# lebrice/blurred-GAN

Measured on AMD Instinct MI355X. Metric: images/sec (G+D+GP step), higher is better.
Workload: dtype f32; 1 GPU; celeba64 64x64x3 batch 256/GPU, blur sigma 5.0 (31 taps), D-step+GP+G-step+Adam; global_batch=256, parallelism=dp1

## Files before the change

blurred-gan_amd/csrc/conv_rows.hip:

```cpp
#include "conv_common.h"
#include <algorithm>
#include <cstdlib>
#include <cstring>
#include <type_traits>

namespace {

typedef float floatx4 __attribute__((ext_vector_type(4)));

struct RowParams {
  const float* A;
  const float* Wt;
  float* C;
  int B, Hi, Wi, Ck, Ho, Wo, N;
  int pt, pl, flip;
  int R, strips;
  int wpr, ipw;
  int epi_mode;
  const float* bias;
  const float* ref;
  const unsigned char* keep;
  size_t keep_elems;
  float alpha, scale;
};

__device__ inline int floordiv(int a, int b) { return a >= 0 ? a / b : -((-a + b - 1) / b); }

__device__ inline float tanh_branchless(float x) {
  float ax = fabsf(x);
  ax = ax > 15.f ? 15.f : ax;
  const float e = __builtin_amdgcn_exp2f(ax * 2.885390081777927f);
  const float big = 1.f - 2.f * __builtin_amdgcn_rcpf(e + 1.f);
  const float x2 = ax * ax;
  const float small = ax * fmaf(x2, fmaf(x2, fmaf(x2, -17.f / 315.f, 2.f / 15.f), -1.f / 3.f), 1.f);
  return copysignf(ax < 0.1f ? small : big, x);
}

template <int KS, int K, int S, int PIXW, int EP>
__global__ __launch_bounds__(PIXW * 4) void conv_rows_scatter_kernel(const RowParams p) {
  constexpr int NTH = PIXW * 4;
  constexpr unsigned kOob = 0x80000000u;
  extern __shared__ __attribute__((aligned(16))) float row_lds[];
  constexpr int AS = 4 * KS + 4;
  float* abuf = row_lds;
  constexpr int PS = PIXW * 17 + 1;
  float* pbuf = row_lds + 2 * PIXW * AS;
  const int tid = threadIdx.x, lane = tid & 63, wave = tid >> 6;
  const int li = lane & 15, kq = lane >> 4;
  const int t = wave % p.wpr, img = wave / p.wpr;
  const int strip = blockIdx.x % p.strips, bgrp = blockIdx.x / p.strips;
  const int Ck = 4 * KS, N = p.N;
  const int y0 = strip * p.R, y1 = min(y0 + p.R, p.Ho);
  const int iy_lo = -floordiv(-(y0 + p.pt - (K - 1)), S);
  const int iy_hi = floordiv(y1 - 1 + p.pt, S);
  const int nrows = iy_hi - iy_lo + 1;
  const int nimg = min(p.ipw, p.B - bgrp * p.ipw);
  const size_t img0 = (size_t)bgrp * p.ipw;
  const __amdgpu_buffer_rsrc_t rsA = __builtin_amdgcn_make_buffer_rsrc(const_cast<float*>(p.A + img0 * p.Hi * p.Wi * Ck), 0,
                                                                        nimg * p.Hi * p.Wi * Ck * 4, 0x00020000);
  const __amdgpu_buffer_rsrc_t rsC = __builtin_amdgcn_make_buffer_rsrc(p.C + img0 * p.Ho * p.Wo * N, 0, nimg * p.Ho * p.Wo * N * 4, 0x00020000);

  float bw[K][KS];
  {
    const int lc = min(li, K * N - 1);
    const int kw = lc / N, n = lc - kw * N;
#pragma unroll
    for (int kh = 0; kh < K; ++kh) {
      const int tap = p.flip ? (K - 1 - kh) * K + (K - 1 - kw) : kh * K + kw;
#pragma unroll
      for (int ks = 0; ks < KS; ++ks) {
        const float w = p.Wt[((size_t)tap * N + n) * Ck + 4 * ks + kq];
        bw[kh][ks] = li < K * N ? w : 0.f;
      }
    }
  }
  floatx4 acc[K];
#pragma unroll
  for (int i = 0; i < K; ++i) acc[i] = floatx4{0.f, 0.f, 0.f, 0.f};

  constexpr int QPR = KS;
  constexpr int NQ = PIXW * QPR / NTH;
  static_assert(NQ >= 1, "Ck >= 16");
  unsigned g_off[NQ], l_off[NQ];
#pragma unroll
  for (int q = 0; q < NQ; ++q) {
    const int f = tid + q * NTH, pix = f / QPR, c4 = f - pix * QPR;
    const int im = pix / p.Wi, ix = pix - im * p.Wi;
    g_off[q] = im < nimg ? (unsigned)(((im * p.Hi * p.Wi + ix) * Ck + c4 * 4) * 4) : kOob;
    l_off[q] = (unsigned)(pix * AS + c4 * 4);
  }
  const int rowB = p.Wi * Ck * 4;
  auto gload = [&](int r, float4 (&g)[NQ]) {
    const int iy = iy_lo + r;
    const bool row_ok = r < nrows && (unsigned)iy < (unsigned)p.Hi;
    const unsigned add = row_ok ? (unsigned)(iy * rowB) : 0u, force = row_ok ? 0u : kOob;
#pragma unroll
    for (int q = 0; q < NQ; ++q)
      g[q] = __builtin_bit_cast(float4, __builtin_amdgcn_raw_buffer_load_b128(rsA, (g_off[q] + add) | force, 0, 0));
  };
  auto lstore = [&](int buf, const float4 (&g)[NQ]) {
#pragma unroll
    for (int q = 0; q < NQ; ++q) *reinterpret_cast<float4*>(abuf + (size_t)buf * PIXW * AS + l_off[q]) = g[q];
  };
  const float* afrag = abuf + ((size_t)img * p.Wi + 16 * t + li) * AS + kq;
  constexpr int NE = (S * (16 / K) + 3) / 4;
  constexpr int NTERM = (K + S - 1) / S;
  int e_src[NE][NTERM];
  unsigned e_dst[NE];
  float e_bias[NE], e_mul[NE];
  int e_n[NE];
  if (tid < 2 * S) pbuf[(size_t)tid * PS + PIXW * 17] = 0.f;
  {
    const int per_img = p.Wo * N;
#pragma unroll
    for (int q = 0; q < NE; ++q) {
      const int e = tid + q * NTH;
      const int im = e / per_img, rem = e - im * per_img;
      const int x = rem / N, n = rem - x * N;
      const bool ok = e < p.ipw * per_img && im < nimg;
      e_dst[q] = ok ? (unsigned)(((im * p.Ho * p.Wo + x) * N + n) * 4) : kOob;
      e_n[q] = n;
      e_bias[q] = ok && p.bias ? p.bias[n] : 0.f;
      e_mul[q] = ok && p.epi_mode == BG_EPI_AFFINE_LRELU ? p.ref[n] : 0.f;
#pragma unroll
      for (int i = 0; i < NTERM; ++i) {
        const int kw = (x + p.pl) % S + i * S;
        const int num = x + p.pl - kw, ix = num / S;
        e_src[q][i] = (ok && kw < K && num >= 0 && ix < p.Wi) ? (im * p.Wi + ix) * 17 + kw * N + n : PIXW * 17;
      }
    }
  }
  const size_t out0 = img0 * p.Ho * p.Wo * N;
  auto pwrite = [&](const floatx4& pacc, int slot) {
    float* pb = pbuf + (size_t)slot * PS;
#pragma unroll
    for (int rr = 0; rr < 4; ++rr) pb[((size_t)img * p.Wi + 16 * t + 4 * kq + rr) * 17 + li] = pacc[rr];
  };
  auto pstore = [&](int slot, int y, bool live) {
    const float* pb = pbuf + (size_t)slot * PS;
    float v[NE];
#pragma unroll
    for (int q = 0; q < NE; ++q) {
      v[q] = pb[e_src[q][0]];
#pragma unroll
      for (int i = 1; i < NTERM; ++i) v[q] += pb[e_src[q][i]];
    }
    const unsigned add = live ? (unsigned)(y * p.Wo * N * 4) : 0u, force = live ? 0u : kOob;
#pragma unroll
    for (int q = 0; q < NE; ++q) {
      const unsigned off = (e_dst[q] + add) | force;
      float o;
      if (EP == 0) {
        o = v[q] + e_bias[q];
      } else if (EP == 1) {
        o = tanh_branchless(v[q] + e_bias[q]);
      } else {
        const bool mine = (off & kOob) == 0;
        o = mine ? bg::apply_epilogue_pre(p, v[q], out0 + (off >> 2), e_bias[q], e_mul[q]) : 0.f;
      }
      __builtin_amdgcn_raw_buffer_store_b32(__builtin_bit_cast(unsigned, o), rsC, off, 0, 0);
    }
  };

  float4 g0[NQ], g1[NQ], g2[NQ], g3[NQ];
  gload(0, g0);
  gload(1, g1);
  gload(2, g2);
  gload(3, g3);
  lstore(0, g0);
  gload(4, g0);
#pragma unroll
  for (int i = 0; i < 4 * NE * S; ++i) __builtin_amdgcn_raw_buffer_store_b32(0u, rsC, kOob + 4u * i, 0, 0);
  int y_prev = 0;
  bool have_prev = false;
  auto flush_prev = [&](int prev_par) {
#pragma unroll
    for (int kh = 0; kh < S; ++kh) {
      const int y = y_prev + kh;
      pstore(prev_par * S + kh, y, have_prev & (y >= y0) & (y < y1));
    }
  };
  auto trip = [&](int r, auto parity, float4 (&g)[NQ]) {
    constexpr int cur = decltype(parity)::value;
    __syncthreads();
    float a[KS];
#pragma unroll
    for (int ks = 0; ks < KS; ++ks) a[ks] = afrag[(size_t)cur * PIXW * AS + 4 * ks];
#pragma unroll
    for (int ks = 0; ks < KS; ++ks)
#pragma unroll
      for (int kh = 0; kh < K; ++kh) acc[kh] = __builtin_amdgcn_mfma_f32_16x16x4f32(a[ks], bw[kh][ks], acc[kh], 0, 0, 0);
    flush_prev(cur ^ 1);
    lstore(cur ^ 1, g);
    gload(r + 5, g);
#pragma unroll
    for (int kh = 0; kh < S; ++kh) pwrite(acc[kh], cur * S + kh);
    y_prev = (iy_lo + r) * S - p.pt;
    have_prev = true;
#pragma unroll
    for (int i = 0; i < K; ++i) acc[i] = i + S < K ? acc[i + S] : floatx4{0.f, 0.f, 0.f, 0.f};
  };
  int r = 0;
  for (; r + 4 <= nrows; r += 4) {
    trip(r, std::integral_constant<int, 0>{}, g1);
    trip(r + 1, std::integral_constant<int, 1>{}, g2);
    trip(r + 2, std::integral_constant<int, 0>{}, g3);
    trip(r + 3, std::integral_constant<int, 1>{}, g0);
  }
  int last_par = 1;
  if (r < nrows) {
    trip(r, std::integral_constant<int, 0>{}, g1);
    last_par = 0;
    if (r + 1 < nrows) {
      trip(r + 1, std::integral_constant<int, 1>{}, g2);
      last_par = 1;
      if (r + 2 < nrows) {
        trip(r + 2, std::integral_constant<int, 0>{}, g3);
        last_par = 0;
      }
    }
  }
  __syncthreads();
  if (last_par == 0) flush_prev(0); else flush_prev(1);
}

template <int K, int S>
int launch_rows(const RowParams& p, dim3 grid, size_t lds, hipStream_t s) {
  const bool wide = p.Wi == 128;
  const int ep = p.epi_mode == BG_EPI_NONE ? 0 : p.epi_mode == BG_EPI_TANH ? 1 : 2;
#define BG_RS2(KSv, EPv) do { if (wide) bg::launch((conv_rows_scatter_kernel<KSv, K, S, 128, EPv>), grid, dim3(512), lds, s, p); \
                              else bg::launch((conv_rows_scatter_kernel<KSv, K, S, 64, EPv>), grid, dim3(256), lds, s, p); } while (0)
#define BG_RS(KSv) do { if (ep == 0) BG_RS2(KSv, 0); else if (ep == 1) BG_RS2(KSv, 1); else BG_RS2(KSv, 2); } while (0)
  switch (p.Ck) {
    case 16: BG_RS(4); return 1;
    case 32: BG_RS(8); return 1;
    case 64: BG_RS(16); return 1;
    default: return 0;
  }
#undef BG_RS
#undef BG_RS2
}

constexpr int kRgHalo = 16;

struct RowGParams {
  const float* A;
  const float* Wt;
  float* C;
  int B, Hi, Wi, Ct, Ho, Wo, N;
  int s, pt, pl, flip;
  int R, strips;
  int epi_mode;
  const float* bias;
  const float* ref;
  const unsigned char* keep;
  size_t keep_elems;
  float alpha, scale;
};

template <int TG, int NT, int K, bool MASK>
__global__ __launch_bounds__(256) void conv_rows_gather_kernel(const RowGParams p) {
  extern __shared__ __attribute__((aligned(16))) float xl[];
  const int tid = threadIdx.x, lane = tid & 63, wave = tid >> 6;
  const int li = lane & 15, kq = lane >> 4;
  const int Ct = p.Ct, N = 16 * NT, st = p.s;
  const int RS = p.Wi * Ct + 2 * kRgHalo;
  const int strip = blockIdx.x % p.strips, b = blockIdx.x / p.strips;
  const int oy0 = strip * p.R, rows = min(p.R, p.Ho - oy0);
  const int nrows_in = (rows - 1) * st + K;

  float bw[K][4][NT];
#pragma unroll
  for (int ks = 0; ks < 4; ++ks) {
    const int i = 4 * ks + kq, kw = i / Ct, ci = i - kw * Ct;
#pragma unroll
    for (int kh = 0; kh < K; ++kh) {
      const int tap = p.flip ? (K - 1 - kh) * K + (K - 1 - kw) : kh * K + kw;
#pragma unroll
      for (int nt = 0; nt < NT; ++nt) bw[kh][ks][nt] = i < K * Ct ? p.Wt[((size_t)tap * N + nt * 16 + li) * Ct + ci] : 0.f;
    }
  }
  const int RL = p.Wi * Ct;
  if ((RL & 3) == 0) {
    const int q4 = RS / 4;
    bg::stage_rows_f4<4>(xl, nrows_in, q4, RS, tid, [&](int r, int c4) -> const float* {
      const int iy = oy0 * st - p.pt + r, e = c4 * 4 - kRgHalo;
      return ((unsigned)iy < (unsigned)p.Hi && (unsigned)e < (unsigned)RL) ? p.A + ((size_t)b * p.Hi + iy) * RL + e : nullptr;
    });
  } else {
    for (int idx = tid; idx < nrows_in * RS; idx += 256) {
      const int r = idx / RS, c = idx - r * RS;
      const int iy = oy0 * st - p.pt + r, e = c - kRgHalo;
      float v = 0.f;
      if ((unsigned)iy < (unsigned)p.Hi && (unsigned)e < (unsigned)RL) v = p.A[((size_t)b * p.Hi + iy) * RL + e];
      xl[idx] = v;
    }
  }
  __syncthreads();

  float e_bias[NT], e_mul[NT];
#pragma unroll
  for (int nt = 0; nt < NT; ++nt) {
    e_bias[nt] = p.bias ? p.bias[nt * 16 + li] : 0.f;
    e_mul[nt] = p.epi_mode == BG_EPI_AFFINE_LRELU ? p.ref[nt * 16 + li] : 1.f;
  }
  const int groups = p.Wo / (16 * TG);
  const int nunits = rows * groups;
  for (int u = wave; u < nunits; u += 4) {
    const int r = u / groups, g = u - r * groups;
    const int oy = oy0 + r, ox0 = g * 16 * TG;
    floatx4 acc[TG][NT];
#pragma unroll
    for (int tg = 0; tg < TG; ++tg)
#pragma unroll
      for (int nt = 0; nt < NT; ++nt) acc[tg][nt] = floatx4{0.f, 0.f, 0.f, 0.f};
    const float* abase = xl + (size_t)(r * st) * RS + kRgHalo + ((ox0 + li) * st - p.pl) * Ct + kq;
#pragma unroll
    for (int kh = 0; kh < K; ++kh) {
      float a[TG][4];
#pragma unroll
      for (int tg = 0; tg < TG; ++tg)
#pragma unroll
        for (int ks = 0; ks < 4; ++ks) a[tg][ks] = abase[(size_t)kh * RS + tg * 16 * st * Ct + 4 * ks];
#pragma unroll
      for (int ks = 0; ks < 4; ++ks)
#pragma unroll
        for (int tg = 0; tg < TG; ++tg)
#pragma unroll
          for (int nt = 0; nt < NT; ++nt) acc[tg][nt] = __builtin_amdgcn_mfma_f32_16x16x4f32(a[tg][ks], bw[kh][ks][nt], acc[tg][nt], 0, 0, 0);
    }
    constexpr bool mask_epi = MASK;
#pragma unroll
    for (int tg = 0; tg < TG; ++tg) {
      const size_t pix0 = ((size_t)b * p.Ho + oy) * p.Wo + ox0 + 16 * tg + 4 * kq;
      unsigned char e_keep[4][NT];
      if (mask_epi) {
#pragma unroll
        for (int rr = 0; rr < 4; ++rr)
#pragma unroll
          for (int nt = 0; nt < NT; ++nt) {
            const size_t idx = (pix0 + rr) * N + nt * 16 + li;
            e_keep[rr][nt] = p.keep[(p.keep_elems == 0 || idx < p.keep_elems) ? idx : 0];
          }
      }
#pragma unroll
      for (int rr = 0; rr < 4; ++rr)
#pragma unroll
        for (int nt = 0; nt < NT; ++nt) {
          const size_t idx = (pix0 + rr) * N + nt * 16 + li;
          if (mask_epi) {
            float v = acc[tg][nt][rr] + e_bias[nt];
            v = v > 0.f ? v : p.alpha * v;
            if (p.keep_elems == 0 || idx < p.keep_elems) v = e_keep[rr][nt] ? v * p.scale : 0.f;
            p.C[idx] = v;
          } else {
            p.C[idx] = bg::apply_epilogue_pre(p, acc[tg][nt][rr], idx, e_bias[nt], e_mul[nt]);
          }
        }
    }
  }
}

template <int K>
int launch_rows_gather(const RowGParams& p, int tg, dim3 grid, size_t lds, hipStream_t s) {
  const int nt = p.N / 16;
  const bool mask = p.epi_mode == BG_EPI_BIAS_LRELU && p.keep != nullptr;
#define BG_RG(TGv, NTv) do { if (mask) bg::launch((conv_rows_gather_kernel<TGv, NTv, K, true>), grid, dim3(256), lds, s, p); \
                             else bg::launch((conv_rows_gather_kernel<TGv, NTv, K, false>), grid, dim3(256), lds, s, p); } while (0)
  if (tg == 1) { if (nt == 1) BG_RG(1, 1); else if (nt == 2) BG_RG(1, 2); else BG_RG(1, 4); }
  else if (tg == 2) { if (nt == 1) BG_RG(2, 1); else if (nt == 2) BG_RG(2, 2); else BG_RG(2, 4); }
  else { if (nt == 1) BG_RG(4, 1); else if (nt == 2) BG_RG(4, 2); else BG_RG(4, 4); }
#undef BG_RG
  return 1;
}

}

namespace bg {

int try_conv_rows_gather(int bwd_data, const float* a, const float* w, float* c, int B, int H, int W, int Cin, int Cout, int k, int s,
                         const bg_epilogue* epi, void* stream, int* taken) {
  *taken = 0;
  static const int off = getenv("BG_NO_ROWS") ? 1 : 0;
  if (off || (k != 5 && k != 3)) return BG_OK;
  RowGParams p;
  memset(&p, 0, sizeof p);
  int Ho, Wo, pt, pl;
  same_pads(H, k, s, &Ho, &pt);
  same_pads(W, k, s, &Wo, &pl);
  if (bwd_data) {
    if (s != 1 || Cout * k > 16 || (Cin != 16 && Cin != 32 && Cin != 64)) return BG_OK;
    p.Hi = H; p.Wi = W; p.Ct = Cout; p.Ho = H; p.Wo = W; p.N = Cin; p.s = 1; p.pt = k - 1 - pt; p.pl = k - 1 - pl; p.flip = 1;
  } else {
    if (Cin * k > 16 || (Cout != 16 && Cout != 32 && Cout != 64)) return BG_OK;
    p.Hi = H; p.Wi = W; p.Ct = Cin; p.Ho = Ho; p.Wo = Wo; p.N = Cout; p.s = s; p.pt = pt; p.pl = pl; p.flip = 0;
  }
  if (p.Wo % 16 != 0) return BG_OK;
  if ((size_t)B * p.Ho * p.Wo * p.N >= (1ull << 31)) return BG_OK;
  const int tiles = p.Wo / 16;
  const int tg = tiles % 4 == 0 ? 4 : (tiles % 2 == 0 ? 2 : 1);
  p.A = a; p.Wt = w; p.C = c; p.B = B;
  static const int rows_r = getenv("BG_ROWSG_R") ? atoi(getenv("BG_ROWSG_R")) : 0;
  p.R = std::min(rows_r ? rows_r : (s == 2 ? 8 : 16), p.Ho);
  p.strips = (int)cdiv(p.Ho, p.R);
  const size_t lds = ((size_t)((p.R - 1) * p.s + k) * (p.Wi * p.Ct + 2 * kRgHalo)) * sizeof(float);
  if (lds > 64 * 1024) return BG_OK;
  p.epi_mode = BG_EPI_NONE; p.alpha = 0.3f; p.scale = 1.f;
  if (epi) {
    BG_REQUIRE(epi->mode >= BG_EPI_NONE && epi->mode <= BG_EPI_AFFINE_LRELU, BG_ERR_UNSUPPORTED, "conv rows: epilogue mode %d", epi->mode);
    BG_REQUIRE(epi->mode != BG_EPI_MUL_GRAD || epi->ref, BG_ERR_NULL, "conv rows: BG_EPI_MUL_GRAD needs ref");
    BG_REQUIRE(epi->mode != BG_EPI_AFFINE_LRELU || (epi->ref && epi->bias), BG_ERR_NULL, "conv rows: BG_EPI_AFFINE_LRELU needs ref and bias");
    p.epi_mode = epi->mode; p.bias = epi->bias; p.ref = epi->ref; p.keep = epi->keep; p.keep_elems = epi->keep_elems; p.alpha = epi->alpha; p.scale = epi->scale;
  }
  const dim3 grid((unsigned)(B * p.strips));
  const double flops = 2.0 * B * (double)Ho * Wo * Cin * Cout * k * k;
  Launch L(stream, bwd_data ? "conv_rows_thin_k_dgrad" : "conv_rows_thin_k_fwd", flops, 0);
  if (k == 5) launch_rows_gather<5>(p, tg, grid, lds, L.s);
  else launch_rows_gather<3>(p, tg, grid, lds, L.s);
  *taken = 1;
  return L.done("conv_rows_gather_kernel");
}



int try_conv_rows(int bwd_data, const float* a, const float* w, float* c, int B, int H, int W, int Cin, int Cout, int k, int s,
                  const bg_epilogue* epi, void* stream, int* taken) {
  *taken = 0;
  static const int off = getenv("BG_NO_ROWS") ? 1 : 0;
  if (off || (k != 5 && k != 3)) return BG_OK;
  RowParams p;
  memset(&p, 0, sizeof p);
  int Ho, Wo, pt, pl;
  same_pads(H, k, s, &Ho, &pt);
  same_pads(W, k, s, &Wo, &pl);
  if (bwd_data) {
    if (Cin * k > 16 || (Cout != 16 && Cout != 32 && Cout != 64)) return BG_OK;
    p.Hi = Ho; p.Wi = Wo; p.Ck = Cout; p.Ho = H; p.Wo = W; p.N = Cin; p.pt = pt; p.pl = pl; p.flip = 0;
  } else {
    if (s != 1 || Cout * k > 16 || (Cin != 16 && Cin != 32 && Cin != 64)) return BG_OK;
    p.Hi = H; p.Wi = W; p.Ck = Cin; p.Ho = H; p.Wo = W; p.N = Cout; p.pt = k - 1 - pt; p.pl = k - 1 - pl; p.flip = 1;
  }
  if (p.Wi != 16 && p.Wi != 32 && p.Wi != 64 && p.Wi != 128) return BG_OK;
  if ((size_t)B * p.Hi * p.Wi * p.Ck >= (1ull << 31) || (size_t)B * p.Ho * p.Wo * p.N >= (1ull << 31)) return BG_OK;
  p.A = a; p.Wt = w; p.C = c; p.B = B;
  static const int rows_r = getenv("BG_ROWS_R") ? atoi(getenv("BG_ROWS_R")) : 0;
  p.R = std::min(rows_r ? rows_r : (s == 1 ? 32 : 16), p.Ho);
  p.strips = (int)cdiv(p.Ho, p.R);
  p.wpr = p.Wi / 16;
  p.ipw = p.Wi == 128 ? 1 : 4 / p.wpr;
  const int pixw = p.Wi == 128 ? 128 : 64;
  if ((long)p.ipw * p.Wo * p.N > (long)((s * (16 / k) + 3) / 4) * pixw * 4) return BG_OK;
  if ((size_t)p.ipw * p.Hi * p.Wi * p.Ck >= (1ull << 29) || (size_t)p.ipw * p.Ho * p.Wo * p.N >= (1ull << 29)) return BG_OK;
  p.epi_mode = BG_EPI_NONE; p.alpha = 0.3f; p.scale = 1.f;
  if (epi) {
    BG_REQUIRE(epi->mode >= BG_EPI_NONE && epi->mode <= BG_EPI_AFFINE_LRELU, BG_ERR_UNSUPPORTED, "conv rows: epilogue mode %d", epi->mode);
    BG_REQUIRE(epi->mode != BG_EPI_MUL_GRAD || epi->ref, BG_ERR_NULL, "conv rows: BG_EPI_MUL_GRAD needs ref");
    BG_REQUIRE(epi->mode != BG_EPI_AFFINE_LRELU || (epi->ref && epi->bias), BG_ERR_NULL, "conv rows: BG_EPI_AFFINE_LRELU needs ref and bias");
    p.epi_mode = epi->mode; p.bias = epi->bias; p.ref = epi->ref; p.keep = epi->keep; p.keep_elems = epi->keep_elems; p.alpha = epi->alpha; p.scale = epi->scale;
  }
  const dim3 grid((unsigned)(cdiv(B, p.ipw) * p.strips));
  const size_t lds = ((size_t)2 * pixw * (p.Ck + 4) + (size_t)2 * s * (pixw * 17 + 1)) * sizeof(float);
  const double flops = 2.0 * B * (double)H * W * Cin * Cout * k * k / (s * s);
  Launch L(stream, bwd_data ? "conv_rows_dgrad" : "conv_rows_fwd", flops, 0);
  int ok;
  if (k == 5) ok = s == 2 ? launch_rows<5, 2>(p, grid, lds, L.s) : launch_rows<5, 1>(p, grid, lds, L.s);
  else ok = s == 2 ? launch_rows<3, 2>(p, grid, lds, L.s) : launch_rows<3, 1>(p, grid, lds, L.s);
  (void)ok;
  *taken = 1;
  return L.done("conv_rows_scatter_kernel");
}

}
```

Baseline: 32500 images/s.

## Make thin-K row-gather conv persistent with double-buffered LDS prefetch and vector epilogues

Turns the row-gather conv into a persistent kernel sized from occupancy, and stages the next strip's input rows into registers while the current strip computes, then writes them into a second LDS buffer. Specialized epilogue variants (bias, bias+lrelu+dropout mask, mul-grad) use buffer loads and 128-bit stores with packed mask bytes instead of scalar per-element stores. It also transposes the MFMA operands so each lane holds four consecutive channels, enabling vector stores. The cost is doubled LDS usage, more template variants, extra alignment guards, and added register pressure.

```diff
diff --git a/blurred-gan_amd/csrc/conv_rows.hip b/blurred-gan_amd/csrc/conv_rows.hip
--- a/blurred-gan_amd/csrc/conv_rows.hip
+++ b/blurred-gan_amd/csrc/conv_rows.hip
@@ -2,11 +2,15 @@
 #include <algorithm>
 #include <cstdlib>
 #include <cstring>
+#include <map>
+#include <mutex>
 #include <type_traits>
+#include <utility>
 
 namespace {
 
 typedef float floatx4 __attribute__((ext_vector_type(4)));
+typedef unsigned uintx4 __attribute__((ext_vector_type(4)));
 
 struct RowParams {
   const float* A;
@@ -242,6 +246,11 @@
 }
 
 constexpr int kRgHalo = 16;
+constexpr int kRgPF = 4;
+constexpr int kRgBias = 0;
+constexpr int kRgLrelu = 1;
+constexpr int kRgMulGrad = 2;
+constexpr int kRgAny = 3;
 
 struct RowGParams {
   const float* A;
@@ -250,6 +259,9 @@
   int B, Hi, Wi, Ct, Ho, Wo, N;
   int s, pt, pl, flip;
   int R, strips;
+  int total;
+  int pre;
+  int ct_rcp;
   int epi_mode;
   const float* bias;
   const float* ref;
@@ -258,119 +270,231 @@
   float alpha, scale;
 };
 
-template <int TG, int NT, int K, bool MASK>
-__global__ __launch_bounds__(256) void conv_rows_gather_kernel(const RowGParams p) {
+template <int TG, int NT, int K, int EP>
+__global__ __launch_bounds__(256, (NT > 2 || EP == kRgAny) ? 1 : ((TG <= 2 || EP == kRgBias) ? 4 : 3)) void conv_rows_gather_kernel(const RowGParams p) {
+  constexpr unsigned kOob = 0x80000000u;
+  constexpr int N = 16 * NT;
   extern __shared__ __attribute__((aligned(16))) float xl[];
-  const int tid = threadIdx.x, lane = tid & 63, wave = tid >> 6;
+  const int tid = threadIdx.x, lane = tid & 63, wave = __builtin_amdgcn_readfirstlane(tid >> 6);
   const int li = lane & 15, kq = lane >> 4;
-  const int Ct = p.Ct, N = 16 * NT, st = p.s;
-  const int RS = p.Wi * Ct + 2 * kRgHalo;
-  const int strip = blockIdx.x % p.strips, b = blockIdx.x / p.strips;
-  const int oy0 = strip * p.R, rows = min(p.R, p.Ho - oy0);
-  const int nrows_in = (rows - 1) * st + K;
+  const int Ct = p.Ct, st = p.s;
+  const int RL = p.Wi * Ct;
+  const int RS = RL + 2 * kRgHalo;
+  const int nrmax = (p.R - 1) * st + K, bufsz = nrmax * RS;
+  constexpr bool pre = EP != kRgAny;
 
   float bw[K][4][NT];
-#pragma unroll
-  for (int ks = 0; ks < 4; ++ks) {
-    const int i = 4 * ks + kq, kw = i / Ct, ci = i - kw * Ct;
-#pragma unroll
-    for (int kh = 0; kh < K; ++kh) {
-      const int tap = p.flip ? (K - 1 - kh) * K + (K - 1 - kw) : kh * K + kw;
-#pragma unroll
-      for (int nt = 0; nt < NT; ++nt) bw[kh][ks][nt] = i < K * Ct ? p.Wt[((size_t)tap * N + nt * 16 + li) * Ct + ci] : 0.f;
-    }
-  }
-  const int RL = p.Wi * Ct;
-  if ((RL & 3) == 0) {
-    const int q4 = RS / 4;
-    bg::stage_rows_f4<4>(xl, nrows_in, q4, RS, tid, [&](int r, int c4) -> const float* {
-      const int iy = oy0 * st - p.pt + r, e = c4 * 4 - kRgHalo;
-      return ((unsigned)iy < (unsigned)p.Hi && (unsigned)e < (unsigned)RL) ? p.A + ((size_t)b * p.Hi + iy) * RL + e : nullptr;
-    });
-  } else {
-    for (int idx = tid; idx < nrows_in * RS; idx += 256) {
-      const int r = idx / RS, c = idx - r * RS;
-      const int iy = oy0 * st - p.pt + r, e = c - kRgHalo;
-      float v = 0.f;
-      if ((unsigned)iy < (unsigned)p.Hi && (unsigned)e < (unsigned)RL) v = p.A[((size_t)b * p.Hi + iy) * RL + e];
-      xl[idx] = v;
-    }
-  }
-  __syncthreads();
-
-  float e_bias[NT], e_mul[NT];
+  {
+    const __amdgpu_buffer_rsrc_t rsW = __builtin_amdgcn_make_buffer_rsrc(const_cast<float*>(p.Wt), 0, K * K * N * Ct * 4, 0x00020000);
+#pragma unroll
+    for (int ks = 0; ks < 4; ++ks) {
+      const int i = 4 * ks + kq, kw = (i * p.ct_rcp) >> 16, ci = i - kw * Ct;
+      const int kwt = p.flip ? K - 1 - kw : kw;
+      const unsigned vo = i < K * Ct ? (unsigned)(((kwt * N + li) * Ct + ci) * 4) : kOob;
+#pragma unroll
+      for (int kh = 0; kh < K; ++kh) {
+        const int kht = p.flip ? K - 1 - kh : kh;
+#pragma unroll
+        for (int nt = 0; nt < NT; ++nt)
+          bw[kh][ks][nt] = __builtin_bit_cast(float, __builtin_amdgcn_raw_buffer_load_b32(rsW, vo, (kht * K * N + nt * 16) * Ct * 4, 0));
+      }
+    }
+  }
+  float4 e_bias[NT], e_mul[NT];
 #pragma unroll
   for (int nt = 0; nt < NT; ++nt) {
-    e_bias[nt] = p.bias ? p.bias[nt * 16 + li] : 0.f;
-    e_mul[nt] = p.epi_mode == BG_EPI_AFFINE_LRELU ? p.ref[nt * 16 + li] : 1.f;
-  }
+    const int c = nt * 16 + 4 * kq;
+    e_bias[nt] = p.bias ? make_float4(p.bias[c], p.bias[c + 1], p.bias[c + 2], p.bias[c + 3]) : make_float4(0.f, 0.f, 0.f, 0.f);
+    e_mul[nt] = (EP == kRgAny && p.epi_mode == BG_EPI_AFFINE_LRELU) ? make_float4(p.ref[c], p.ref[c + 1], p.ref[c + 2], p.ref[c + 3])
+                                                                     : make_float4(1.f, 1.f, 1.f, 1.f);
+  }
+
+  unsigned gl_off[kRgPF];
+  if constexpr (pre) {
+    const int q4 = RL >> 2, dr = 256 / q4, dc = 256 - dr * q4;
+    int r = tid / q4, c4 = tid - r * q4;
+#pragma unroll
+    for (int i = 0; i < kRgPF; ++i) {
+      const unsigned packed = (unsigned)(r * q4 + c4) | ((unsigned)(r * (RS >> 2) + kRgHalo / 4 + c4) << 16);
+      gl_off[i] = r < nrmax ? packed : (unsigned)(kRgHalo / 4) << 16;
+      r += dr; c4 += dc;
+      if (c4 >= q4) { c4 -= q4; ++r; }
+    }
+  }
+  float4 pf[kRgPF];
+  auto prefetch = [&](int w) {
+    const bool ok = w < p.total;
+    const int b = ok ? w / p.strips : 0, strip = w - b * p.strips;
+    const __amdgpu_buffer_rsrc_t rsA = __builtin_amdgcn_make_buffer_rsrc(const_cast<float*>(p.A + (size_t)b * p.Hi * RL), 0, p.Hi * RL * 4, 0x00020000);
+    const unsigned add = (unsigned)((strip * p.R * st - p.pt) * RL * 4), force = ok ? 0u : kOob;
+#pragma unroll
+    for (int i = 0; i < kRgPF; ++i)
+      pf[i] = __builtin_bit_cast(float4, __builtin_amdgcn_raw_buffer_load_b128(rsA, (((gl_off[i] & 0xffffu) << 4) + add) | force, 0, 0));
+  };
+  auto stash = [&](int buf) {
+#pragma unroll
+    for (int i = 0; i < kRgPF; ++i) *reinterpret_cast<float4*>(xl + buf * bufsz + (gl_off[i] >> 16) * 4) = pf[i];
+  };
+
+  int w = blockIdx.x, buf = 0;
+  if constexpr (pre) {
+    prefetch(w);
+    for (int idx = tid; idx < 2 * nrmax * 2 * kRgHalo; idx += 256) {
+      const int e = idx & (kRgHalo - 1), side = (idx / kRgHalo) & 1, r = idx / (2 * kRgHalo);
+      xl[r * RS + (side ? kRgHalo + RL : 0) + e] = 0.f;
+    }
+    stash(0);
+    __syncthreads();
+  }
+  const int img = p.Ho * p.Wo * N;
   const int groups = p.Wo / (16 * TG);
-  const int nunits = rows * groups;
-  for (int u = wave; u < nunits; u += 4) {
-    const int r = u / groups, g = u - r * groups;
-    const int oy = oy0 + r, ox0 = g * 16 * TG;
-    floatx4 acc[TG][NT];
-#pragma unroll
-    for (int tg = 0; tg < TG; ++tg)
-#pragma unroll
-      for (int nt = 0; nt < NT; ++nt) acc[tg][nt] = floatx4{0.f, 0.f, 0.f, 0.f};
-    const float* abase = xl + (size_t)(r * st) * RS + kRgHalo + ((ox0 + li) * st - p.pl) * Ct + kq;
-#pragma unroll
-    for (int kh = 0; kh < K; ++kh) {
-      float a[TG][4];
+  for (; w < p.total; w += gridDim.x) {
+    const int b = w / p.strips, strip = w - b * p.strips;
+    const int oy0 = strip * p.R, rows = min(p.R, p.Ho - oy0);
+    if constexpr (pre) {
+      prefetch(w + gridDim.x);
+    } else {
+      const int nrows_in = (rows - 1) * st + K;
+      if ((RL & 3) == 0) {
+        const int q4 = RS / 4;
+        bg::stage_rows_f4<4>(xl, nrows_in, q4, RS, tid, [&](int r, int c4) -> const float* {
+          const int iy = oy0 * st - p.pt + r, e = c4 * 4 - kRgHalo;
+          return ((unsigned)iy < (unsigned)p.Hi && (unsigned)e < (unsigned)RL) ? p.A + ((size_t)b * p.Hi + iy) * RL + e : nullptr;
+        });
+      } else {
+        for (int idx = tid; idx < nrows_in * RS; idx += 256) {
+          const int r = idx / RS, c = idx - r * RS;
+          const int iy = oy0 * st - p.pt + r, e = c - kRgHalo;
+          float v = 0.f;
+          if ((unsigned)iy < (unsigned)p.Hi && (unsigned)e < (unsigned)RL) v = p.A[((size_t)b * p.Hi + iy) * RL + e];
+          xl[idx] = v;
+        }
+      }
+      __syncthreads();
+    }
+    const float* xb = xl + buf * bufsz;
+    const size_t ib = (size_t)b * img;
+    const __amdgpu_buffer_rsrc_t rsC = __builtin_amdgcn_make_buffer_rsrc(p.C + ib, 0, img * 4, 0x00020000);
+    const size_t cov = p.keep ? (p.keep_elems ? p.keep_elems : (size_t)p.B * img) : 0;
+    const unsigned cov_img = cov > ib ? (unsigned)min(cov - ib, (size_t)img) : 0u;
+    const __amdgpu_buffer_rsrc_t rsK = __builtin_amdgcn_make_buffer_rsrc(
+        p.keep ? const_cast<unsigned char*>(p.keep) + ib : reinterpret_cast<unsigned char*>(p.C), 0, (int)cov_img, 0x00020000);
+    const __amdgpu_buffer_rsrc_t rsR = __builtin_amdgcn_make_buffer_rsrc(
+        EP == kRgMulGrad ? const_cast<float*>(p.ref) + ib : p.C, 0, EP == kRgMulGrad ? img * 4 : 0, 0x00020000);
+
+    const int nunits = rows * groups;
+    for (int u = wave; u < nunits; u += 4) {
+      const int r = u / groups, g = u - r * groups;
+      const int oy = oy0 + r, ox0 = g * 16 * TG;
+      const unsigned off0 = (unsigned)((((oy * p.Wo + ox0 + li) * N) + 4 * kq) * 4);
+      constexpr bool early = EP == kRgLrelu;
+      unsigned e_keep[TG][NT];
+      float4 e_ref[TG][NT];
+      auto request = [&](int tg) {
+#pragma unroll
+        for (int nt = 0; nt < NT; ++nt) {
+          const unsigned eo = off0 + (unsigned)((tg * 16 * N + nt * 16) * 4);
+          e_keep[tg][nt] = __builtin_amdgcn_raw_buffer_load_b32(rsK, eo >> 2, 0, 0);
+          if (EP == kRgMulGrad) e_ref[tg][nt] = __builtin_bit_cast(float4, __builtin_amdgcn_raw_buffer_load_b128(rsR, eo, 0, 0));
+        }
+      };
+      if (early) {
+#pragma unroll
+        for (int tg = 0; tg < TG; ++tg) request(tg);
+      }
+      floatx4 acc[TG][NT];
 #pragma unroll
       for (int tg = 0; tg < TG; ++tg)
 #pragma unroll
-        for (int ks = 0; ks < 4; ++ks) a[tg][ks] = abase[(size_t)kh * RS + tg * 16 * st * Ct + 4 * ks];
-#pragma unroll
-      for (int ks = 0; ks < 4; ++ks)
+        for (int nt = 0; nt < NT; ++nt) acc[tg][nt] = floatx4{0.f, 0.f, 0.f, 0.f};
+      const float* abase = xb + (size_t)(r * st) * RS + kRgHalo + ((ox0 + li) * st - p.pl) * Ct + kq;
+#pragma unroll
+      for (int kh = 0; kh < K; ++kh) {
+        float a[TG][4];
 #pragma unroll
         for (int tg = 0; tg < TG; ++tg)
 #pragma unroll
-          for (int nt = 0; nt < NT; ++nt) acc[tg][nt] = __builtin_amdgcn_mfma_f32_16x16x4f32(a[tg][ks], bw[kh][ks][nt], acc[tg][nt], 0, 0, 0);
-    }
-    constexpr bool mask_epi = MASK;
-#pragma unroll
-    for (int tg = 0; tg < TG; ++tg) {
-      const size_t pix0 = ((size_t)b * p.Ho + oy) * p.Wo + ox0 + 16 * tg + 4 * kq;
-      unsigned char e_keep[4][NT];
-      if (mask_epi) {
-#pragma unroll
-        for (int rr = 0; rr < 4; ++rr)
-#pragma unroll
-          for (int nt = 0; nt < NT; ++nt) {
-            const size_t idx = (pix0 + rr) * N + nt * 16 + li;
-            e_keep[rr][nt] = p.keep[(p.keep_elems == 0 || idx < p.keep_elems) ? idx : 0];
+          for (int ks = 0; ks < 4; ++ks) a[tg][ks] = abase[(size_t)kh * RS + tg * 16 * st * Ct + 4 * ks];
+#pragma unroll
+        for (int ks = 0; ks < 4; ++ks)
+#pragma unroll
+          for (int tg = 0; tg < TG; ++tg)
+#pragma unroll
+            for (int nt = 0; nt < NT; ++nt) acc[tg][nt] = __builtin_amdgcn_mfma_f32_16x16x4f32(bw[kh][ks][nt], a[tg][ks], acc[tg][nt], 0, 0, 0);
+      }
+#pragma unroll
+      for (int tg = 0; tg < TG; ++tg) {
+        if (!early && (EP == kRgLrelu || EP == kRgMulGrad)) request(tg);
+#pragma unroll
+        for (int nt = 0; nt < NT; ++nt) {
+          const unsigned eo = off0 + (unsigned)((tg * 16 * N + nt * 16) * 4);
+          const floatx4 v = acc[tg][nt];
+          const float4 bi = e_bias[nt];
+          float4 o;
+          if (EP == kRgBias) {
+            o = make_float4(v[0] + bi.x, v[1] + bi.y, v[2] + bi.z, v[3] + bi.w);
+          } else if (EP == kRgLrelu || EP == kRgMulGrad) {
+            const bool covered = (eo >> 2) < cov_img;
+            const unsigned k4 = covered ? e_keep[tg][nt] : 0x01010101u;
+            const float sc = covered ? p.scale : 1.f;
+            if (EP == kRgLrelu) {
+              float t0 = v[0] + bi.x, t1 = v[1] + bi.y, t2 = v[2] + bi.z, t3 = v[3] + bi.w;
+              t0 = t0 > 0.f ? t0 : p.alpha * t0; t1 = t1 > 0.f ? t1 : p.alpha * t1; t2 = t2 > 0.f ? t2 : p.alpha * t2; t3 = t3 > 0.f ? t3 : p.alpha * t3;
+              o = make_float4((k4 & 0xffu) ? t0 * sc : 0.f, (k4 & 0xff00u) ? t1 * sc : 0.f, (k4 & 0xff0000u) ? t2 * sc : 0.f,
+                              (k4 & 0xff000000u) ? t3 * sc : 0.f);
+            } else {
+              const float4 rf = e_ref[tg][nt];
+              float f0 = rf.x > 0.f ? 1.f : p.alpha, f1 = rf.y > 0.f ? 1.f : p.alpha, f2 = rf.z > 0.f ? 1.f : p.alpha, f3 = rf.w > 0.f ? 1.f : p.alpha;
+              f0 = (k4 & 0xffu) ? f0 * sc : 0.f; f1 = (k4 & 0xff00u) ? f1 * sc : 0.f; f2 = (k4 & 0xff0000u) ? f2 * sc : 0.f;
+              f3 = (k4 & 0xff000000u) ? f3 * sc : 0.f;
+              o = make_float4((v[0] + bi.x) * f0, (v[1] + bi.y) * f1, (v[2] + bi.z) * f2, (v[3] + bi.w) * f3);
+            }
+          } else {
+            o = bg::apply_epilogue4(p, make_float4(v[0], v[1], v[2], v[3]), ib + (eo >> 2), &e_bias[nt].x, &e_mul[nt].x);
           }
-      }
-#pragma unroll
-      for (int rr = 0; rr < 4; ++rr)
-#pragma unroll
-        for (int nt = 0; nt < NT; ++nt) {
-          const size_t idx = (pix0 + rr) * N + nt * 16 + li;
-          if (mask_epi) {
-            float v = acc[tg][nt][rr] + e_bias[nt];
-            v = v > 0.f ? v : p.alpha * v;
-            if (p.keep_elems == 0 || idx < p.keep_elems) v = e_keep[rr][nt] ? v * p.scale : 0.f;
-            p.C[idx] = v;
-          } else {
-            p.C[idx] = bg::apply_epilogue_pre(p, acc[tg][nt][rr], idx, e_bias[nt], e_mul[nt]);
-          }
+          __builtin_amdgcn_raw_buffer_store_b128(__builtin_bit_cast(uintx4, o), rsC, eo, 0, 0);
         }
-    }
-  }
+      }
+    }
+    if constexpr (pre) {
+      buf ^= 1;
+      stash(buf);
+    }
+    __syncthreads();
+  }
+}
+
+int rows_gather_slots(const void* kern, size_t lds) {
+  static const int forced = getenv("BG_ROWSG_WGS") ? atoi(getenv("BG_ROWSG_WGS")) : 0;
+  if (forced > 0) return forced;
+  static std::mutex mu;
+  static std::map<std::pair<const void*, size_t>, int> cache;
+  std::lock_guard<std::mutex> lock(mu);
+  auto it = cache.find({kern, lds});
+  if (it != cache.end()) return it->second;
+  int dev = 0, cus = 0, per_cu = 0;
+  if (hipGetDevice(&dev) != hipSuccess || hipDeviceGetAttribute(&cus, hipDeviceAttributeMultiprocessorCount, dev) != hipSuccess || cus <= 0) cus = 256;
+  if (hipOccupancyMaxActiveBlocksPerMultiprocessor(&per_cu, kern, 256, lds) != hipSuccess || per_cu <= 0) per_cu = 1;
+  const int slots = cus * std::min(per_cu, 8);
+  cache[{kern, lds}] = slots;
+  return slots;
 }
 
 template <int K>
-int launch_rows_gather(const RowGParams& p, int tg, dim3 grid, size_t lds, hipStream_t s) {
+int launch_rows_gather(const RowGParams& p, int tg, int ep, size_t lds, hipStream_t s) {
   const int nt = p.N / 16;
-  const bool mask = p.epi_mode == BG_EPI_BIAS_LRELU && p.keep != nullptr;
-#define BG_RG(TGv, NTv) do { if (mask) bg::launch((conv_rows_gather_kernel<TGv, NTv, K, true>), grid, dim3(256), lds, s, p); \
-                             else bg::launch((conv_rows_gather_kernel<TGv, NTv, K, false>), grid, dim3(256), lds, s, p); } while (0)
+#define BG_RG1(TGv, NTv, EPv) do { void (*kern)(const RowGParams) = conv_rows_gather_kernel<TGv, NTv, K, EPv>;                     \
+                                   const int slots = rows_gather_slots(reinterpret_cast<const void*>(kern), lds);                  \
+                                   bg::launch(kern, dim3((unsigned)std::min(p.total, slots)), dim3(256), lds, s, p); } while (0)
+#define BG_RG(TGv, NTv) do { if (K == 5 && ep == kRgBias) BG_RG1(TGv, NTv, (K == 5 ? kRgBias : kRgAny));             \
+                             else if (K == 5 && ep == kRgLrelu) BG_RG1(TGv, NTv, (K == 5 ? kRgLrelu : kRgAny));      \
+                             else if (K == 5 && ep == kRgMulGrad) BG_RG1(TGv, NTv, (K == 5 ? kRgMulGrad : kRgAny));  \
+                             else BG_RG1(TGv, NTv, kRgAny); } while (0)
   if (tg == 1) { if (nt == 1) BG_RG(1, 1); else if (nt == 2) BG_RG(1, 2); else BG_RG(1, 4); }
   else if (tg == 2) { if (nt == 1) BG_RG(2, 1); else if (nt == 2) BG_RG(2, 2); else BG_RG(2, 4); }
-  else { if (nt == 1) BG_RG(4, 1); else if (nt == 2) BG_RG(4, 2); else BG_RG(4, 4); }
+  else { if (nt == 1) BG_RG(4, 1); else if (nt == 2) BG_RG(4, 2); else BG_RG1(4, 4, kRgAny); }
 #undef BG_RG
+#undef BG_RG1
   return 1;
 }
 
@@ -397,14 +521,18 @@
   }
   if (p.Wo % 16 != 0) return BG_OK;
   if ((size_t)B * p.Ho * p.Wo * p.N >= (1ull << 31)) return BG_OK;
+  if ((size_t)p.Ho * p.Wo * p.N >= (1ull << 29) || (size_t)p.Hi * p.Wi * p.Ct >= (1ull << 28)) return BG_OK;
   const int tiles = p.Wo / 16;
   const int tg = tiles % 4 == 0 ? 4 : (tiles % 2 == 0 ? 2 : 1);
   p.A = a; p.Wt = w; p.C = c; p.B = B;
   static const int rows_r = getenv("BG_ROWSG_R") ? atoi(getenv("BG_ROWSG_R")) : 0;
-  p.R = std::min(rows_r ? rows_r : (s == 2 ? 8 : 16), p.Ho);
+  p.R = std::min(rows_r > 0 ? rows_r : (s == 2 ? 8 : 16), p.Ho);
   p.strips = (int)cdiv(p.Ho, p.R);
-  const size_t lds = ((size_t)((p.R - 1) * p.s + k) * (p.Wi * p.Ct + 2 * kRgHalo)) * sizeof(float);
-  if (lds > 64 * 1024) return BG_OK;
+  p.total = B * p.strips;
+  p.ct_rcp = 65536 / p.Ct + 1;
+  const int nrmax = (p.R - 1) * p.s + k, RL = p.Wi * p.Ct;
+  const size_t lds1 = ((size_t)nrmax * (RL + 2 * kRgHalo)) * sizeof(float);
+  if (lds1 > 64 * 1024) return BG_OK;
   p.epi_mode = BG_EPI_NONE; p.alpha = 0.3f; p.scale = 1.f;
   if (epi) {
     BG_REQUIRE(epi->mode >= BG_EPI_NONE && epi->mode <= BG_EPI_AFFINE_LRELU, BG_ERR_UNSUPPORTED, "conv rows: epilogue mode %d", epi->mode);
@@ -412,11 +540,23 @@
     BG_REQUIRE(epi->mode != BG_EPI_AFFINE_LRELU || (epi->ref && epi->bias), BG_ERR_NULL, "conv rows: BG_EPI_AFFINE_LRELU needs ref and bias");
     p.epi_mode = epi->mode; p.bias = epi->bias; p.ref = epi->ref; p.keep = epi->keep; p.keep_elems = epi->keep_elems; p.alpha = epi->alpha; p.scale = epi->scale;
   }
-  const dim3 grid((unsigned)(B * p.strips));
+  const bool mask_used = p.keep && (p.epi_mode == BG_EPI_BIAS_LRELU || p.epi_mode == BG_EPI_MUL_GRAD);
+  if (mask_used && (!aligned16(p.keep) || p.keep_elems % 4 != 0)) return BG_OK;
+  if (p.epi_mode == BG_EPI_MUL_GRAD && !aligned16(p.ref)) return BG_OK;
+  p.pre = RL % 4 == 0 && (size_t)nrmax * (RL / 4) <= (size_t)kRgPF * 256 && 2 * lds1 <= 64 * 1024;
+  int ep = kRgAny;
+  if (p.pre && k == 5) {
+    if (p.epi_mode == BG_EPI_NONE) ep = kRgBias;
+    else if (p.epi_mode == BG_EPI_BIAS_LRELU) ep = kRgLrelu;
+    else if (p.epi_mode == BG_EPI_MUL_GRAD) ep = kRgMulGrad;
+  }
+  p.pre = ep != kRgAny;
+  const size_t lds = p.pre ? 2 * lds1 : lds1;
+  const int tgl = (ep != kRgAny && p.N == 64 && tg == 4) ? 2 : tg;
   const double flops = 2.0 * B * (double)Ho * Wo * Cin * Cout * k * k;
   Launch L(stream, bwd_data ? "conv_rows_thin_k_dgrad" : "conv_rows_thin_k_fwd", flops, 0);
-  if (k == 5) launch_rows_gather<5>(p, tg, grid, lds, L.s);
-  else launch_rows_gather<3>(p, tg, grid, lds, L.s);
+  if (k == 5) launch_rows_gather<5>(p, tgl, ep, lds, L.s);
+  else launch_rows_gather<3>(p, tgl, ep, lds, L.s);
   *taken = 1;
   return L.done("conv_rows_gather_kernel");
 }
```

Result: no change. 32680 images/s, median of 6 (+0.6%).
